# NagsTheProgrammer/WindGNN

Hardware: AMD Instinct MI355X
Metric: windows/sec (fwd+bwd) 34-node seq24 GCN-GRU (higher is better)
Workload: dtype f16x3(split-fp32); 1 GPU; S=34 stations, T=24, F=13, H=102, B=4096 windows/GPU; step = forward + MSE + backward + grad all-reduce (N>1) + Adam; fp32 I/O; global_batch=4096, parallelism=dp1, math=f16x3, collective=none (one rank)

## Files before the change

windgnn_amd/csrc/api.hip:

```cpp
#include <atomic>
#include <cmath>
#include <cstdlib>
#include <mutex>

#include "common.h"
#include "../../include/windgnn_optim.h"
#include "../../include/windgnn_sched.h"

namespace {

inline size_t rup(size_t x, size_t a) { return (x + a - 1) / a * a; }

struct Layout {
  size_t BT, I, Ip, G3, Gp, H, Hp;
  size_t Id;
  int np_g3, np_i;
  size_t ws_GI, ws_g, ws_planes_f, ws_Ylast, ws_xtail_f, ws_xtail_b, fwd_floats;
  size_t st_g, st_gates, st_yp, stash_floats;
  size_t ws_dGI, ws_dGH, ws_dg, ws_part_ih, ws_part_hh, ws_gcnpart, ws_planes_b, ws_scales, ws_dY, bwd_floats;
  size_t prep_f, prep_b, prep_floats;
  int prep_kind;
  int sk_ih, sk_hh;
  bool tn_merge;
  bool x3, gen_gcn, gen_gru, g32, g32tn;
// ... 400 lines not shown
}

int fwd_recurrence(const Fwd& f) {
  const wgnn_dims* d = f.d;
  const FwdCall& c = f.c;
  const Layout& L = f.L;
  const wgnn_params* p = c.p;
  const float y_mul = c.wind_max - c.wind_min, y_add = c.wind_min;
  const bool hn_only = c.state && !f.Y;
  float* Y = (float*)f.Y;
  const void* labels = f.sf ? c.labels : nullptr;
  float* stats = f.sf ? f.sf + L.st_stats : nullptr;
  float* hprev = (f.sf && (L.g32tn || c.sst)) ? f.sf + L.st_hprev : nullptr;
  int rc;
  if (L.x3 && !L.gen_gru) {
    if (c.last)
      return launch_grux_fwd(d->B, d->T, d->H, f.GI, (int)L.Gp, p->w_hh, p->b_hh, c.last, nullptr, nullptr, f.full, f.status,
                             nullptr, nullptr, 0, 1, y_mul, y_add, f.st);
    if (c.state) {
      const int lo = hn_only && d->io == WGNN_IO_F32;
      return launch_grux_fwd(d->B, d->T, d->H, f.GI, (int)L.Gp, p->w_hh, p->b_hh, lo ? (void*)c.hn : f.Y, nullptr, nullptr,
                             f.full, f.status, nullptr, nullptr, d->io, lo, 1.f, 0.f, f.st, c.h0, lo ? nullptr : c.hn);
    }
    rc = launch_grux_fwd(d->B, d->T, d->H, f.GI, (int)L.Gp, p->w_hh, p->b_hh, f.Y, f.gates, f.sf ? f.sf + L.st_yp : nullptr,
                         f.full, f.status, labels, stats, d->io, 0, 1.f, 0.f, f.st, c.h0, c.hn, c.sst ? L.plane_rows : 0);
  } else if (L.rec32) {
    if (c.last)
      return launch_gru_fwd(d->B, d->T, d->H, f.GI, (int)L.Gp, p->w_hh, p->b_hh, c.last, nullptr, nullptr, nullptr, nullptr, 0,
                            1, y_mul, y_add, f.st);
    if (c.state)
      return launch_gru_fwd(d->B, d->T, d->H, f.GI, (int)L.Gp, p->w_hh, p->b_hh, hn_only ? c.hn : Y, nullptr, nullptr, nullptr,
                            nullptr, 0, hn_only ? 1 : 0, 1.f, 0.f, f.st, c.h0, hn_only ? nullptr : c.hn);
    rc = launch_gru_fwd(d->B, d->T, d->H, f.GI, (int)L.Gp, p->w_hh, p->b_hh, Y, f.gates, (const float*)labels, stats, hprev,
                        L.hq, 0, 1.f, 0.f, f.st, c.h0, c.hn);
  } else if (L.small) {
    rc = launch_gru_small_fwd(d->B, d->T, d->H, f.GI, (int)L.Gp, p->w_hh, p->b_hh, Y, f.gates, hprev, L.hq,
                              (const float*)labels, stats, f.st, c.h0, c.hn);
  } else if (L.x3) {
    rc = launch_split_weight2(p->w_hh, (int)L.G3, (int)L.H, 0, p->b_hh, (int)L.H, f.ws + L.ws_hhp_f, L.np_g3, (int)L.Hp,
                              f.status, f.st);
    if (rc == WGNN_OK)
      rc = launch_gru_gen_fwd_x3(d->B, d->T, d->H, f.GI, (int)L.Gp, f.ws + L.ws_hhp_f, L.np_g3, p->b_hh, Y, f.gates,
                                 f.sf ? f.sf + L.st_yp : f.ws + L.ws_yp, f.ws + L.ws_gh, f.ws + L.ws_kp_f, f.ws + L.ws_hc,
                                 f.full, f.st, c.h0, c.sst ? L.plane_rows : 0);
  } else {
    rc = launch_gru_gen_fwd(d->B, d->T, d->H, f.GI, (int)L.Gp, p->w_hh, p->b_hh, Y, f.gates, f.ws + L.ws_gh, f.st, c.h0);
  }
  if (rc != WGNN_OK) return rc;
// ... 133 lines not shown
  if (L.gen_gru)
    return launch_gru_gen_bwd(d->B, d->T, d->H, p->w_hh, b.Y, dY, gates, b.dGI, b.dGH, (int)L.Gp, b.ws + L.ws_dhz,
                              b.ws + L.ws_dhw, b.st, sb);
  if (L.small)
    return launch_gru_small_bwd(d->B, d->T, d->H, p->w_hh, b.Y, b.fused_loss ? nullptr : dY, b.fused_loss ? labels : nullptr,
                                gates, b.dGI, b.dGH, (int)L.Gp, stats, (int64_t)L.BT * L.H, c.grad_scale, c.loss, b.status,
                                b.st, sb);
  return launch_gru_bwd(d->B, d->T, d->H, p->w_hh, b.Y, b.fused_loss ? nullptr : dY, b.fused_loss ? labels : nullptr, gates,
                        b.sf + L.st_GI, (int)L.Gp, b.dGI, (int)L.Gp, L.dghn ? b.dGH : nullptr, L.dghn ? nullptr : b.dGH, stats,
                        (int64_t)L.BT * L.H, c.grad_scale, c.loss, b.status, b.st, sb);
}

int bwd_weights(const Bwd& b, int prods, int r0, int rows) {
  const wgnn_dims* d = b.d;
  const Layout& L = b.L;
  float* part_ih = b.ws + L.ws_part_ih;
  float* part_hh = b.ws + L.ws_part_hh;
  const bool sst = b.c.sst;
  int rc = WGNN_OK;
  if (L.x3) {
    const _Float16* dGIh = (const _Float16*)b.dGI + r0;
    const _Float16* dGHh = (const _Float16*)b.dGH + r0;
    const _Float16* gh = (const _Float16*)b.gact;
    const _Float16* yph = (const _Float16*)(b.sf + L.st_yp);
    const _Float16* ypl = yph + L.plane_rows * L.Hp;
    const size_t PG = L.BT * L.Gp;
    TnProd hh = {};
    hh.lda = (int)L.Gp; hh.Bhi = yph; hh.Blo = ypl; hh.ldb = (int)L.Hp; hh.shift_T = d->T; hh.splitk = L.sk_hh;
    hh.partial = part_hh; hh.Nout = (int)L.H + 1; hh.x3 = b.full; hh.per_window = sst;
    if (L.dghn) {
      hh.Ahi = dGIh; hh.Alo = L.dgi1 ? nullptr : dGIh + PG; hh.Mout = L.m_hh;
      hh.A2hi = dGHh; hh.A2lo = L.dgi1 ? nullptr : dGHh + L.BT * (size_t)L.hn; hh.lda2 = L.hn; hh.msplit = L.msplit;
      hh.b_stream = true;
    } else {
      hh.Ahi = dGHh; hh.Alo = L.gen2p ? nullptr : dGHh + PG; hh.Mout = rows;
    }
    const bool one_pass_ih = L.dgi1 || L.gen2p;
    TnProd ih = {};
    ih.Ahi = dGIh; ih.Alo = one_pass_ih ? dGIh : dGIh + PG; ih.lda = (int)L.Gp;
    ih.Bhi = gh; ih.Blo = gh + L.BT * L.Ip; ih.ldb = (int)L.Ip; ih.splitk = L.sk_ih;
    ih.partial = part_ih; ih.Mout = rows; ih.Nout = (int)L.I + 1; ih.x3 = b.full && !one_pass_ih; ih.b_stream = true;
    auto one = [&](const TnProd& p) {
      return launch_pgemm_tn(p.Ahi, p.Alo, p.lda, p.Bhi, p.Blo, p.ldb, p.shift_T, (int)L.BT, p.splitk, p.partial, p.Mout, p.Nout,
                             p.x3, p.A2hi, p.A2lo, p.lda2, p.msplit, b.st, p.b_stream, p.per_window);
    };
    if (prods == (WGNN_ROWS_IH | WGNN_ROWS_HH) && L.tn_merge && opt(WGNN_OPT_TN_MERGED) && pgemm_tn2_covers(ih, hh)) {
      rc = launch_pgemm_tn2(ih, hh, (int)L.BT, b.st);
    } else {
      if (prods & WGNN_ROWS_HH) {
        rc = one(hh);
        if (rc != WGNN_OK) return rc;
      }
      if (prods & WGNN_ROWS_IH) rc = one(ih);
    }
  } else {
    const float* hp = b.sf + L.st_hprev;
    if (prods & WGNN_ROWS_HH) {
      if (L.g32tn && L.dghn)
        rc = launch_gemm32_tn(b.dGI, (int)L.Gp, hp, L.hq, (int)L.BT, L.sk_hh, part_hh, L.m_hh, (int)L.H + 1, b.dGH, L.hn,
                              L.msplit, b.st);
      else if (L.g32tn)
        rc = launch_gemm32_tn(b.dGH, (int)L.Gp, hp, L.hq, (int)L.BT, L.sk_hh, part_hh, rows, (int)L.H + 1, nullptr, 0, 0, b.st);
      else {
        GemmArgs a = {};
        a.A = b.dGH + r0; a.lda = (int)L.Gp; a.a_kcontig = 0;
        a.B = b.Y; a.ldb = (int)L.H; a.b_kcontig = 0; a.ones_col = 1; a.shift_T = d->T;
        if (sst) { a.B = hp; a.ldb = L.hq; a.shift_T = 0; }
        a.M = rows; a.N = (int)L.H + 1; a.K = (int)L.BT;
        a.splitk = L.sk_hh; a.partial = part_hh;
        rc = launch_gemm_f32(a, b.st);
// ... 110 lines not shown

int rows_align(const wgnn_dims* d, const Layout& L) {
  if (!L.gen_gru || d->math == WGNN_MATH_F16) return 0;
  return L.x3 ? TN_BM : 128;
}

int check_rows(const wgnn_dims* d, const Layout& L, int which, int row0, int rows) {
  if ((which & ~(WGNN_ROWS_IH | WGNN_ROWS_HH | WGNN_ROWS_STATE)) != 0 ||
      ((which & 3) != WGNN_ROWS_IH && (which & 3) != WGNN_ROWS_HH))
    return WGNN_ERR_SHAPE;
  if (which & WGNN_ROWS_STATE) return WGNN_ERR_UNSUPPORTED;
  const int al = rows_align(d, L);
  if (al == 0) return WGNN_ERR_UNSUPPORTED;
  const int64_t end = (int64_t)row0 + rows;
  if (row0 < 0 || rows < 1 || end > (int64_t)L.G3 || row0 % al != 0 || (end % al != 0 && end != (int64_t)L.G3))
    return WGNN_ERR_SHAPE;
  return WGNN_OK;
}

}

int opt_big_gemm() { return opt(WGNN_OPT_BIG_GEMM); }

int series_plan(const wgnn_dims* df, const wgnn_dims* dr, SeriesPlan* sp) {
  int rc = check_dims(df);
  if (rc == WGNN_OK) rc = check_dims(dr);
  if (rc != WGNN_OK) return rc;
  const Layout Lf = make_layout(df, false, SER_FRONT), Lr = make_layout(dr, false, SER_REC);
  if ((int64_t)Lf.BT * (int64_t)Lf.Gp >= (1ll << 31)) return WGNN_ERR_SHAPE;
  sp->ws_front = Lf.fwd_floats > Lf.bwd_floats ? Lf.fwd_floats : Lf.bwd_floats;
  sp->ws_rec = Lr.fwd_floats > Lr.bwd_floats ? Lr.fwd_floats : Lr.bwd_floats;
  sp->st_front = Lf.stash_floats;
  sp->st_rec = Lr.stash_floats;
  sp->st_g = Lf.BT * Lf.Ip; sp->st_GI = Lf.BT * Lf.Gp;
  sp->st_gates = gru_gates_floats(dr->B, dr->T, dr->H);
  sp->st_hprev = Lr.g32tn ? Lr.BT * (size_t)Lr.hq : 0;
  return WGNN_OK;
}

namespace {

int series_forward(const wgnn_dims* df, const wgnn_dims* dr, int stride, const float* A, const float* Xs, const wgnn_params* p,
                   float* Y, float* last, float wind_min, float wind_max, void* stash, void* workspace, const SeriesPlan& sp,
                   void* stream, const float* Ls, int64_t ls_rows, float* loss_buf, const int* starts) {
  const int last_start = df->T - dr->T;
  const Layout Lf = make_layout(df, false, SER_FRONT), Lr = make_layout(dr, false, SER_REC);
// ... 449 lines not shown
```

windgnn_amd/csrc/common.h:

```cpp
#pragma once
#include <hip/hip_runtime.h>
#include <stdint.h>

#include "../../include/windgnn.h"

typedef float f32x4 __attribute__((ext_vector_type(4)));
typedef float f32x16 __attribute__((ext_vector_type(16)));

#define WGNN_WAVE 64

static inline int cdiv_i(int a, int b) { return (a + b - 1) / b; }
static inline size_t align_up(size_t x, size_t a) { return (x + a - 1) / a * a; }

#define WGNN_CHECK_LAUNCH()                              \
  do {                                                   \
    if (hipGetLastError() != hipSuccess) return WGNN_ERR_HIP; \
  } while (0)

__device__ __forceinline__ f32x4 mfma16(float a, float b, f32x4 c) {
  return __builtin_amdgcn_mfma_f32_16x16x4f32(a, b, c, 0, 0, 0);
}
__device__ __forceinline__ f32x16 mfma32(float a, float b, f32x16 c) {
  return __builtin_amdgcn_mfma_f32_32x32x2f32(a, b, c, 0, 0, 0);
}
// ... 117 lines not shown
                     hipStream_t st);
int launch_gcnx2_bwd(int ntiles, int S, const float* A, const void* X, int io, const float* W1, const float* b1,
                     const float* W2, const void* g_planes, int ldg, const void* dg, int ld_dg ,
                     bool dg16 , const float* scales, int scale_in, float* partial, bool x3,
                     void* xtail_scratch, hipStream_t st);
bool gcngi_supported(int S, int H, bool x3);
int launch_gcngi_fwd(int ntiles, int S, const float* A, const void* X, int io, const float* W1, const float* b1,
                     const float* W2, const float* b2, void* g_planes, int ldg, int stash_planes, const void* Bplanes,
                     int Np, void* GI, int ldgi, int N, bool x3, unsigned* status, void* xtail_scratch, hipStream_t st);
bool gcn_any_supported(int S, int Fi, int Fo);
size_t gcn_any_bwd_partial_floats(int ntiles, int Fi, int Fo);
int launch_gcn_any_fwd(int ntiles, int S, int Fi, int Fo, const float* A, const float* X, const float* W, const float* b, float* out,
                       hipStream_t st);
int launch_gcn_any_bwd(int ntiles, int S, int Fi, int Fo, const float* A, const float* X, const float* W, const float* out,
                       const float* dout, float* dW, float* db, float* dX, float* partial, hipStream_t st);
int launch_pack_g(const float* gin, size_t rows, int I, float* g, int ld, hipStream_t st);
int launch_unpack_dg(const float* dg, size_t rows, int I, int ld, float* out, hipStream_t st);
bool pgemm_nt256_wanted(int M, int N, int Kp);
int launch_pgemm_nt256(const void* Aimg_hi, const void* Aimg_lo, int M, int k0, int klen, const void* Bplanes, int Np,
                       size_t bplane, float* C, int ldc, int N, bool accumulate, hipStream_t st);
size_t pgemm_nt256_aimg_bytes(int M, int N, int Kp, int planes);
int launch_pgemm_repack_a(const void* Ahi, const void* Alo, int lda, int M, int Kp, void* img, hipStream_t st);
int opt_big_gemm();
__host__ __device__ __forceinline__ size_t bimg_off(int n, int k, int Np) {
  return ((size_t)(k >> 5) * (size_t)(Np >> 4) + (size_t)(n >> 4)) * 512 + (size_t)(((k >> 3) & 3) * 128 + (n & 15) * 8 + (k & 7));
}
int launch_split_weight2(const float* W, int R, int C, int transpose, const float* bias, int bias_col, void* planes,
                         int Rp, int Cp, unsigned* status, hipStream_t st);
int pgemm_nt_np(int N);
int pgemm_tn_tiles(int Mout, int Nout);
size_t pgemm_tn_partial_floats(int Mout, int Nout, int splitk);
size_t pgemm_nt_kpart_floats(int M, int ldc, int Kp);
int launch_pgemm_nt(const void* Ahi, const void* Alo, int lda, int M, int Kp, const void* Bplanes, int Np, float* C,
                    int ldc, int N, const float* s_out, bool x3, float* kpart, hipStream_t st, bool out16 = false,
                    void* aimg = nullptr );
int launch_pgemm_tn(const void* Ahi, const void* Alo, int lda, const void* Bhi, const void* Blo, int ldb, int shift_T,
                    int K, int splitk, float* partial, int Mout, int Nout, bool x3, const void* A2hi, const void* A2lo,
                    int lda2, int msplit, hipStream_t st, bool b_stream = false ,
                    bool per_window = false );
struct TnProd {
  const void *Ahi, *Alo; int lda;
  const void *Bhi, *Blo; int ldb;
  int shift_T, splitk;
  float* partial;
  int Mout, Nout;
  bool x3;
  const void *A2hi, *A2lo; int lda2, msplit;
  bool b_stream, per_window;
};
bool pgemm_tn2_covers(const TnProd& ih, const TnProd& hh);
int launch_pgemm_tn2(const TnProd& ih, const TnProd& hh, int K, hipStream_t st);
size_t gcn_csr_bwd_partial_floats();
int launch_gcn2_csr_fwd(int ntiles, int S, int nnz, const void* csr, const float* X, const float* W1, const float* b1,
                        const float* W2, const float* b2, float* h1, float* g, void* g_planes, size_t ldg, bool x3,
                        unsigned* status, hipStream_t st);
int launch_gcn2_csr_bwd(int ntiles, int S, int nnz, const void* csr, const float* X, const float* W2, const float* h1,
                        const float* g, const void* g_hi, size_t ldg, const float* dg, size_t ld_dg,
                        const float* scales, float* du, float* partial, float* dW1, float* db1, float* dW2, float* db2,
                        hipStream_t st);
int launch_gru_gen_fwd_x3(int B, int T, int H, const float* GI, int ldgi, const void* whh_planes, int np_g3,
                          const float* bhh, float* Y, float* gates, void* y_planes, float* gh, float* kpart, void* hc,
                          bool x3, hipStream_t st, const float* h0 = nullptr,
                          size_t plane_rows = 0 );
int launch_h0_planes(int B, int H, int Hp, const float* h0, void* hi, void* lo, hipStream_t st);
int launch_gru_gen_bwd_x3(int B, int T, int H, const void* whhT_planes, int np_h, const float* Y, const float* dY,
                          const float* gates, const float* scales, void* dgi_planes, void* dgh_planes, int ldd,
                          float* dhz, float* dhw, float* kpart, void* dc, bool x3, hipStream_t st,
                          const BwdState* state = nullptr);
int launch_gru_gen_fwd(int B, int T, int H, const float* GI, int ldgi, const float* Whh, const float* bhh, float* Y,
                       float* gates, float* gh, hipStream_t st, const float* h0 = nullptr);
int launch_gru_gen_bwd(int B, int T, int H, const float* Whh, const float* Y, const float* dY, const float* gates,
                       float* dGI, float* dGH, int ldd, float* dhz, float* dhw, hipStream_t st,
                       const BwdState* state = nullptr);
// ... 137 lines not shown
```

windgnn_amd/csrc/pgemm.hip:

```cpp
#include <string>

#include "common.h"

typedef _Float16 h8 __attribute__((ext_vector_type(8)));
typedef _Float16 h4 __attribute__((ext_vector_type(4)));
typedef __fp16 fh4 __attribute__((__vector_size__(4 * sizeof(__fp16))));
typedef unsigned int u32x4 __attribute__((ext_vector_type(4)));

namespace {

constexpr int NT_BM = 192, NT_WAVES = 12;

__device__ __forceinline__ int swz16(int row) { return (4 - (row >> 2)) & 3; }
__device__ __forceinline__ int sw16_off(int row, int c) { return row * 64 + ((c ^ swz16(row)) << 4); }

__device__ __forceinline__ f32x4 mfma_q(h8 a, h8 b, f32x4 c) {
  return __builtin_amdgcn_mfma_f32_16x16x32_f16(a, b, c, 0, 0, 0);
}

constexpr int nt_a_slot(bool x3, bool alo) { return ((x3 && alo) ? 2 : 1) * NT_BM * 64; }
constexpr int nt_b_slot(int T, bool x3) { return (x3 ? 2 : 1) * 32 * T * 64; }
constexpr int nt_a_depth(int T, bool x3, bool alo) {
  return (!x3 && 3 * nt_a_slot(x3, alo) + 2 * nt_b_slot(T, x3) <= 156 * 1024) ? 3 : 2;
}
constexpr size_t nt_smem(int T, bool x3, bool alo) {
  return (size_t)nt_a_depth(T, x3, alo) * nt_a_slot(x3, alo) + 2 * (size_t)nt_b_slot(T, x3);
}

template <int T, bool X3, bool ALO, bool OUT16>
__global__ void __launch_bounds__(64 * NT_WAVES) pgemm_nt_kernel(const _Float16* __restrict__ Ahi,
                                                                const _Float16* __restrict__ Alo, int lda, int M,
                                                                int Kp, const _Float16* __restrict__ Bpl, int Np,
                                                                float* __restrict__ C, int ldc, int N,
                                                                const float* __restrict__ s_out_p, int nm, int nsl,
                                                                size_t bplane, int kc_len, int kc_first,
                                                                size_t cstride, int accumulate) {
  {
    const int k0 = (kc_first + (int)blockIdx.y) * kc_len;
    Ahi += k0;
    Alo += k0;
// ... 217 lines not shown
  for (int j = 0; j < T; ++j) {
    const int col = n0 + BNW * wn + 16 * j + r16;
    if (col >= N) continue;
#pragma unroll
    for (int i = 0; i < 2; ++i)
#pragma unroll
      for (int r = 0; r < 4; ++r) {
        const int row = m0 + 32 * wm + 16 * i + 4 * c4 + r;
        if (row < M) {
          float* dst = C + (size_t)row * ldc + col;
          const float v = acc[i][j][r] * s_out;
          *dst = accumulate ? *dst + v : v;
        }
      }
  }
}


__device__ __forceinline__ int tn_g(int stride32, int r) {
  const int u = stride32 & 7;
  return u == 0 ? (r & 7) : (u == 4 ? ((r >> 1) & 3) : ((r >> 2) & 1));
}

template <int T, bool X3, bool A2, bool ALO, bool PW = false>
__device__ __forceinline__ void pgemm_tn_tile(const _Float16* __restrict__ Ahi, const _Float16* __restrict__ Alo, int lda,
                                              const _Float16* __restrict__ Bhi, const _Float16* __restrict__ Blo, int ldb,
                                              int shift_T, int K, int kchunk, float* __restrict__ partial, int Mout,
                                              int Nout, int nNb, const _Float16* __restrict__ A2hi,
                                              const _Float16* __restrict__ A2lo, int lda2, int msplit, int b_stream,
                                              const int z, const int tile, const int ntile) {
  constexpr int BM = TN_BM, BN = 32 * T;
  constexpr int ARB = BM * 2, BRB = BN * 2;
  constexpr int A_PL = 32 * ARB, B_PL = 32 * BRB, STAGE = 2 * A_PL + 2 * B_PL;
  constexpr int PL = X3 ? 2 : 1;
  constexpr int PLA = (X3 && ALO) ? 2 : 1;
  constexpr int AP = A_PL / 1024, BP = B_PL / 1024;
  constexpr int NPIECE = PLA * AP + PL * BP, NIT = (NPIECE + TN_WAVES - 1) / TN_WAVES;
  constexpr int ACH = ARB / 16, BCH = BRB / 16;
  extern __shared__ __attribute__((aligned(16))) char smem[];
  const int tid = threadIdx.x, lane = tid & 63;
  const int wave = __builtin_amdgcn_readfirstlane(tid >> 6);
  const int wm = wave & 3, wn = wave >> 2;
  const int mb = tile / nNb, nb = tile % nNb;
  const int m0 = mb * BM, n0 = nb * BN;
  const int kbeg = z * kchunk, kend = min(K, kbeg + kchunk);
  const int nk = kend > kbeg ? (kend - kbeg + 31) / 32 : 0;

  f32x4 acc[5][T];
#pragma unroll
  for (int i = 0; i < 5; ++i)
#pragma unroll
    for (int j = 0; j < T; ++j) acc[i][j] = f32x4{0.f, 0.f, 0.f, 0.f};

  const _Float16* base[NIT];
  int ld[NIT], dst[NIT], prow[NIT], pcol[NIT];
  bool on[NIT], isb[NIT];
#pragma unroll
  for (int it = 0; it < NIT; ++it) {
    const int p = wave + TN_WAVES * it;
    on[it] = p < NPIECE;
    const int pp = on[it] ? p : 0;
    isb[it] = pp >= PLA * AP;
    if (!isb[it]) {
      const int plane = pp / AP, q = 64 * (pp % AP) + lane;
      const int row = q / ACH, pos = q % ACH;
      const int col = m0 + 8 * (pos ^ (2 * tn_g(ARB / 32, row)));
      base[it] = plane ? Alo : Ahi;
      ld[it] = lda;
      prow[it] = row;
      pcol[it] = col < lda ? col : 0;
      if (A2 && col >= msplit) {
        base[it] = plane ? A2lo : A2hi;
        ld[it] = lda2;
        pcol[it] = col - msplit < lda2 ? col - msplit : 0;
      }
      dst[it] = plane * A_PL + (pp % AP) * 1024;
    } else {
      const int q2 = pp - PLA * AP;
      const int plane = q2 / BP, q = 64 * (q2 % BP) + lane;
      const int row = q / BCH, pos = q % BCH;
      const int col = n0 + 8 * (pos ^ (2 * tn_g(BRB / 32, row)));
      base[it] = plane ? Blo : Bhi;
      ld[it] = ldb;
      prow[it] = row;
      pcol[it] = col < ldb ? col : 0;
      dst[it] = 2 * A_PL + plane * B_PL + (q2 % BP) * 1024;
    }
  }
  typedef __attribute__((address_space(3))) void lds_void;
  typedef __attribute__((address_space(1))) const void glb_void;
  auto dma_stage = [&](char* st, int k0) {
#pragma unroll
    for (int it = 0; it < NIT; ++it)
      if (on[it]) {
        int k = min(k0 + prow[it], kend - 1);
        if (isb[it] && shift_T > 0) k = (k % shift_T) != 0 ? k - 1 : (PW ? K + k / shift_T : K);
        if (isb[it] && b_stream)
          __builtin_amdgcn_global_load_lds((glb_void*)(base[it] + (size_t)k * ld[it] + pcol[it]),
                                           (lds_void*)(st + dst[it]), 16, 0, 2);
        else
          __builtin_amdgcn_global_load_lds((glb_void*)(base[it] + (size_t)k * ld[it] + pcol[it]),
                                           (lds_void*)(st + dst[it]), 16, 0, 0);
      }
  };

  const int x = lane >> 4, q4 = (lane & 15) >> 2, p4 = lane & 3;
  const int r1 = 4 * x + q4;
  const int gA = 2 * tn_g(ARB / 32, r1), gB = 2 * tn_g(BRB / 32, r1);
  int a_off[5], b_off[T];
#pragma unroll
  for (int i = 0; i < 5; ++i) a_off[i] = r1 * ARB + 16 * ((2 * (5 * wm + i) + (p4 >> 1)) ^ gA) + 8 * (p4 & 1);
#pragma unroll
  for (int j = 0; j < T; ++j)
    b_off[j] = 2 * A_PL + r1 * BRB + 16 * ((2 * (T * wn + j) + (p4 >> 1)) ^ gB) + 8 * (p4 & 1);
  typedef __attribute__((address_space(3))) fh4 lds_fh4;
  auto trread = [&](const char* p0, int rb) -> h8 {
    const fh4 v0 = __builtin_amdgcn_ds_read_tr16_b64_v4f16((lds_fh4*)p0);
    const fh4 v1 = __builtin_amdgcn_ds_read_tr16_b64_v4f16((lds_fh4*)(p0 + 16 * rb));
    const h4 w0 = __builtin_bit_cast(h4, v0), w1 = __builtin_bit_cast(h4, v1);
    h8 r;
    r[0] = w0[0]; r[1] = w0[1]; r[2] = w0[2]; r[3] = w0[3];
    r[4] = w1[0]; r[5] = w1[1]; r[6] = w1[2]; r[7] = w1[3];
    return r;
  };
  auto compute = [&](const char* cur) {
    h8 ah[5], al[5];
#pragma unroll
    for (int i = 0; i < 5; ++i) {
      ah[i] = trread(cur + a_off[i], ARB);
      al[i] = ah[i];
      if (X3 && ALO) al[i] = trread(cur + A_PL + a_off[i], ARB);
    }
#pragma unroll
    for (int j = 0; j < T; ++j) {
      const h8 bh = trread(cur + b_off[j], BRB);
      if (X3) {
        const h8 bl = trread(cur + B_PL + b_off[j], BRB);
#pragma unroll
        for (int i = 0; i < 5; ++i) {
          if (ALO) acc[i][j] = mfma_q(al[i], bh, acc[i][j]);
          acc[i][j] = mfma_q(ah[i], bl, acc[i][j]);
        }
      }
#pragma unroll
      for (int i = 0; i < 5; ++i) acc[i][j] = mfma_q(ah[i], bh, acc[i][j]);
    }
  };

  if (nk > 0) dma_stage(smem, kbeg);
  for (int kt = 0; kt < nk; ++kt) {
    char* cur = smem + (kt & 1) * STAGE;
    asm volatile("s_waitcnt vmcnt(0)" ::: "memory");
    __builtin_amdgcn_s_barrier();
    if (kt + 1 < nk) dma_stage(smem + ((kt + 1) & 1) * STAGE, kbeg + 32 * (kt + 1));
    const int rows = kend - (kbeg + 32 * kt);
    if (rows < 32) {
      const u32x4 zero = {0u, 0u, 0u, 0u};
      for (int c = tid; c < (32 - rows) * ACH; c += 64 * TN_WAVES) {
        *(u32x4*)(cur + rows * ARB + 16 * c) = zero;
        if (X3 && ALO) *(u32x4*)(cur + A_PL + rows * ARB + 16 * c) = zero;
      }
      __syncthreads();
    }
    compute(cur);
  }

  float* P = partial + (((size_t)z * ntile + tile) * TN_WAVES + wave) * (5 * T * 256) + lane * 4;
#pragma unroll
  for (int i = 0; i < 5; ++i)
#pragma unroll
    for (int j = 0; j < T; ++j) {
      *(f32x4*)(P + (i * T + j) * 256) = acc[i][j];
    }
}

template <int T, bool X3, bool A2, bool ALO, bool PW = false>
__global__ void __launch_bounds__(64 * TN_WAVES) pgemm_tn_kernel(const _Float16* __restrict__ Ahi,
                                                                const _Float16* __restrict__ Alo, int lda,
                                                                const _Float16* __restrict__ Bhi,
                                                                const _Float16* __restrict__ Blo, int ldb,
                                                                int shift_T, int K, int kchunk,
                                                                float* __restrict__ partial, int Mout, int Nout,
                                                                int nNb, const _Float16* __restrict__ A2hi,
                                                                const _Float16* __restrict__ A2lo, int lda2,
                                                                int msplit, int b_stream) {
  pgemm_tn_tile<T, X3, A2, ALO, PW>(Ahi, Alo, lda, Bhi, Blo, ldb, shift_T, K, kchunk, partial, Mout, Nout, nNb, A2hi, A2lo,
                                    lda2, msplit, b_stream, (int)blockIdx.x, (int)blockIdx.y, (int)gridDim.y);
}

struct TnRole {
  const _Float16 *Ahi, *Alo, *Bhi, *Blo, *A2hi, *A2lo;
  float* partial;
  int lda, ldb, lda2, shift_T, K, kchunk, Mout, Nout, nNb, msplit, b_stream, splitk, ntile;
};
template <int TI, int TH, int MODE, bool PW>
__global__ void __launch_bounds__(64 * TN_WAVES) pgemm_tn2_kernel(const TnRole ih, const TnRole hh) {
  const int item = (int)blockIdx.x;
  if (item < ih.splitk * ih.ntile)
    pgemm_tn_tile<TI, MODE == 0, false, true, false>(ih.Ahi, ih.Alo, ih.lda, ih.Bhi, ih.Blo, ih.ldb, ih.shift_T, ih.K, ih.kchunk,
                                                     ih.partial, ih.Mout, ih.Nout, ih.nNb, ih.A2hi, ih.A2lo, ih.lda2, ih.msplit,
                                                     ih.b_stream, item % ih.splitk, item / ih.splitk, ih.ntile);
  __syncthreads();
  if (item < hh.splitk * hh.ntile)
    pgemm_tn_tile<TH, MODE != 2, true, MODE != 1, PW>(hh.Ahi, hh.Alo, hh.lda, hh.Bhi, hh.Blo, hh.ldb, hh.shift_T, hh.K, hh.kchunk,
                                                      hh.partial, hh.Mout, hh.Nout, hh.nNb, hh.A2hi, hh.A2lo, hh.lda2, hh.msplit,
                                                      hh.b_stream, item % hh.splitk, item / hh.splitk, hh.ntile);
}

__global__ void split_weight2_kernel(const float* __restrict__ W, int R, int C, int transpose,
                                     const float* __restrict__ bias, int bias_col, _Float16* hi, _Float16* lo,
                                     int Rp, int Cp, unsigned* status) {
  typedef _Float16 h8v __attribute__((ext_vector_type(8)));
  const size_t pi = (size_t)blockIdx.x * blockDim.x + threadIdx.x;
  if (pi >= (size_t)Rp * Cp / 8) return;
  const int tile = (int)(pi >> 6), within = (int)(pi & 63);
  const int kt = tile / (Rp >> 4), nt = tile % (Rp >> 4);
  const int r = 16 * nt + (within & 15), c0 = 32 * kt + 8 * (within >> 4);
  float v[8];
  if (transpose) {
#pragma unroll
    for (int k = 0; k < 8; ++k) v[k] = (c0 + k < R && r < C) ? W[(size_t)(c0 + k) * C + r] : 0.f;
  } else if (r < R && c0 + 7 < C && (((size_t)r * C + c0) & 3) == 0) {
    const f32x4 a = *(const f32x4*)(W + (size_t)r * C + c0), b = *(const f32x4*)(W + (size_t)r * C + c0 + 4);
#pragma unroll
    for (int k = 0; k < 4; ++k) { v[k] = a[k]; v[4 + k] = b[k]; }
  } else {
#pragma unroll
    for (int k = 0; k < 8; ++k) {
      const int c = c0 + k;
// ... 238 lines not shown
  case t: return launch_tn_t<t>(Ahi, Alo, lda, Bhi, Blo, ldb, shift_T, K, splitk, partial, Mout, Nout, x3, nNb, A2hi, A2lo, \
                                lda2, msplit, st, b_stream, per_window);
    TN_CASE(1) TN_CASE(2) TN_CASE(3) TN_CASE(4) TN_CASE(5) TN_CASE(6) TN_CASE(7)
#undef TN_CASE
  }
  return WGNN_ERR_SHAPE;
}

namespace {
int tn2_mode(const TnProd& ih, const TnProd& hh) {
  const bool ih3 = ih.x3 && ih.Alo, hh3 = hh.x3 && hh.Alo, hh2 = hh.x3 && !hh.Alo;
  if (ih3 && hh3) return 0;
  if (!ih.x3 && hh2) return 1;
  if (!ih.x3 && !hh.x3) return 2;
  return -1;
}

template <int TI, int TH>
int launch_tn2_t(const TnProd& pi, const TnProd& ph, int K, int mode, int nNi, int nNh, hipStream_t st) {
  auto role = [K](const TnProd& p, int nNb) {
    TnRole r;
    const bool alo = p.Alo != nullptr;
    r.Ahi = (const _Float16*)p.Ahi; r.Alo = (const _Float16*)(alo ? p.Alo : p.Ahi);
    r.Bhi = (const _Float16*)p.Bhi; r.Blo = (const _Float16*)p.Blo;
    r.A2hi = (const _Float16*)p.A2hi; r.A2lo = (const _Float16*)(alo ? p.A2lo : p.A2hi);
    r.partial = p.partial;
    r.lda = p.lda; r.ldb = p.ldb; r.lda2 = p.lda2; r.shift_T = p.shift_T; r.K = K;
    r.kchunk = cdiv_i(cdiv_i(K, p.splitk), 32) * 32;
    r.Mout = p.Mout; r.Nout = p.Nout; r.nNb = nNb; r.msplit = p.msplit; r.b_stream = p.b_stream ? 1 : 0;
    r.splitk = p.splitk; r.ntile = cdiv_i(p.Mout, TN_BM) * nNb;
    return r;
  };
  const TnRole ri = role(pi, nNi), rh = role(ph, nNh);
  constexpr int TMAX = TI > TH ? TI : TH;
  const size_t smem = 2 * (size_t)(2 * 32 * 2 * (TN_BM + 32 * TMAX));
  auto bytes = [K](const TnProd& p) {
    return ((p.x3 && p.Alo) ? 4.0 : 2.0) * (double)K * p.Mout + (p.x3 ? 4.0 : 2.0) * (double)K * p.Nout +
           4.0 * (double)p.splitk * p.Mout * p.Nout;
  };
  const double fl = 2.0 * K * ((double)pi.Mout * pi.Nout + (double)ph.Mout * ph.Nout), by = bytes(pi) + bytes(ph);
  static const std::string base = "pgemm_tn_kernel<" + std::to_string(TI) + "+" + std::to_string(TH);
  static const std::string names[3] = {base + ">", base + ",x2>", base + ",f16>"};
  const int ni = ri.splitk * ri.ntile, nh = rh.splitk * rh.ntile;
  const dim3 grid(ni > nh ? ni : nh), block(64 * TN_WAVES);
#define TN2_GO(MODE, PWV)                                                                                        \
  do {                                                                                                           \
    static std::atomic<unsigned long long> done_{0};                                                             \
    if (ensure_dyn_smem((const void*)pgemm_tn2_kernel<TI, TH, MODE, PWV>, smem, done_) != WGNN_OK) return WGNN_ERR_HIP; \
    PROF_LAUNCH(names[MODE].c_str(), fl, by, st,                                                                 \
                hipLaunchKernelGGL((pgemm_tn2_kernel<TI, TH, MODE, PWV>), grid, block, smem, st, ri, rh));       \
  } while (0)
  switch (2 * mode + (ph.per_window ? 1 : 0)) {
    case 0: TN2_GO(0, false); break;
    case 1: TN2_GO(0, true); break;
    case 2: TN2_GO(1, false); break;
    case 3: TN2_GO(1, true); break;
    case 4: TN2_GO(2, false); break;
    case 5: TN2_GO(2, true); break;
    default: return WGNN_ERR_UNSUPPORTED;
  }
#undef TN2_GO
  WGNN_CHECK_LAUNCH();
  return WGNN_OK;
}
}

bool pgemm_tn2_covers(const TnProd& ih, const TnProd& hh) {
  int nNb, T;
  tn_shape(hh.Nout, nNb, T);
  return tn2_mode(ih, hh) >= 0 && !ih.A2hi && ih.shift_T == 0 && !ih.per_window && hh.A2hi && T <= 4 && ih.splitk >= 1 &&
         hh.splitk >= 1;
}

int launch_pgemm_tn2(const TnProd& ih, const TnProd& hh, int K, hipStream_t st) {
  if (!pgemm_tn2_covers(ih, hh)) return WGNN_ERR_UNSUPPORTED;
  if (ih.lda % 8 != 0 || ih.ldb % 8 != 0 || hh.lda % 8 != 0 || hh.ldb % 8 != 0 || K < 1) return WGNN_ERR_SHAPE;
  if (hh.per_window && hh.shift_T < 1) return WGNN_ERR_SHAPE;
  if (hh.lda2 % 8 != 0 || hh.msplit % 8 != 0 || hh.msplit > hh.lda) return WGNN_ERR_SHAPE;
  int nNi, TI, nNh, TH;
  tn_shape(ih.Nout, nNi, TI);
  tn_shape(hh.Nout, nNh, TH);
  const int mode = tn2_mode(ih, hh);
  switch (4 * (TI - 1) + (TH - 1)) {
#define TN2_CASE(ti, th) \
  case 4 * (ti - 1) + (th - 1): return launch_tn2_t<ti, th>(ih, hh, K, mode, nNi, nNh, st);
#define TN2_ROW(ti) TN2_CASE(ti, 1) TN2_CASE(ti, 2) TN2_CASE(ti, 3) TN2_CASE(ti, 4)
    TN2_ROW(1) TN2_ROW(2) TN2_ROW(3) TN2_ROW(4) TN2_ROW(5) TN2_ROW(6) TN2_ROW(7)
#undef TN2_ROW
#undef TN2_CASE
  }
  return WGNN_ERR_SHAPE;
}
```

windgnn_amd/functional.py:

```python
from __future__ import annotations

import ctypes as C
from typing import Sequence

import torch

from . import _lib

PARAM_ORDER = ("conv1.weight", "conv1.bias", "conv2.weight", "conv2.bias",
               "gru.weight_ih_l0", "gru.weight_hh_l0", "gru.bias_ih_l0", "gru.bias_hh_l0")


_IO_OF = {torch.float32: _lib.IO_F32, torch.float16: _lib.IO_F16, torch.bfloat16: _lib.IO_BF16}


def _require_gpu(*tensors: torch.Tensor, io_ok: bool = False) -> None:
    for t in tensors:
        if not t.is_cuda:
            raise RuntimeError(
                "windgnn_amd runs on an MI355X (HIP) only: got a %s tensor. There is no CPU fallback; "
                "use the oracle under oracle/ for CPU checks." % t.device)
        if t.dtype != torch.float32 and not (io_ok and t.dtype in _IO_OF):
            raise RuntimeError("windgnn_amd: expected float32 tensors, got %s" % t.dtype)

# ... 142 lines not shown
    _require_gpu(*params)
    _require_contiguous(X=X, labels=labels, params=params)
    if X.dim() != 4:
        raise RuntimeError("windgnn_amd: X must be [B, T, S, 13], got %s" % (tuple(X.shape),))
    BX, T, S, F = X.shape
    B = BX if B is None else B
    A, fmt, nnz = _adj(A, S)
    H = params[5].shape[1]
    for name, t in (("h0", h0), ("h_n", h_n)):
        if t is None:
            continue
        _require_gpu(t)
        _require_contiguous(**{name: t})
        if tuple(t.shape) != (B, H) or t.device != X.device:
            raise RuntimeError("windgnn_amd: %s must be [B, H] = [%d, %d] float32 on %s, got %s on %s"
                               % (name, B, H, X.device, tuple(t.shape), t.device))
    d = _lib.Dims(B, T, S, F, H, math, fmt, nnz, _IO_OF[X.dtype])
    ws, ws_bytes = _workspace(d, X.device, refused="wgnn_workspace_bytes(B=%d,T=%d,S=%d,F=%d,H=%d,math=%d,io=%s)"
                              % (B, T, S, F, H, math, X.dtype))
    return A, d, ws, ws_bytes


def gcn_gru_forward_raw(A, X, params: Sequence[torch.Tensor], math=_lib.MATH_F32, want_stash=True, labels=None,
                        prepared=None):
    lib = _lib.load()
    A, d, ws, ws_bytes = _forward_setup(A, X, params, math, labels=labels)
    B, T, H = d.B, d.T, d.H
    stash = torch.empty(lib.wgnn_stash_bytes(C.byref(d)), dtype=torch.uint8, device=X.device) if want_stash else None
    Y = torch.empty(B, T, H, dtype=X.dtype, device=X.device)
    ps = _params_struct(_lib.Params, params, prepared)
    if labels is not None:
        _require_gpu(labels, io_ok=True)
        if labels.dtype != X.dtype:
            raise RuntimeError("windgnn_amd: labels are %s but X is %s (one I/O type per call)" % (labels.dtype, X.dtype))
        if labels.numel() != Y.numel() or not want_stash:
            raise RuntimeError("windgnn_amd: wgnn_fwd_loss needs a stash and labels of Y's size, got %s vs %s"
                               % (tuple(labels.shape), tuple(Y.shape)))
        rc = lib.wgnn_fwd_loss(C.byref(d), _ptr(A), _ptr(X), C.byref(ps), _ptr(labels), _ptr(Y),
                               _stash_ptr(stash), _ptr(ws), ws_bytes, _stream())
        _lib.check(rc, "wgnn_fwd_loss")
        return Y, stash, d
    rc = lib.wgnn_fwd(C.byref(d), _ptr(A), _ptr(X), C.byref(ps), _ptr(Y), _stash_ptr(stash), _ptr(ws), ws_bytes, _stream())
    _lib.check(rc, "wgnn_fwd")
    return Y, stash, d


def gcn_gru_state(A, X, params: Sequence[torch.Tensor], math=_lib.MATH_F32, h0=None, want_y=True, h_n=None):
    lib = _lib.load()
    A, d, ws, ws_bytes = _forward_setup(A, X, params, math, h0=h0, h_n=h_n)
    B, T, H = d.B, d.T, d.H
    Y = torch.empty(B, T, H, dtype=X.dtype, device=X.device) if want_y else None
# ... 404 lines not shown
```

Before: 5.666 million windows/s.

## Feed hh weight-gradient GEMM directly from fp32 Y, skipping split-plane stash

In the x3 (split-fp16) path the forward GRU no longer writes hi/lo fp16 planes of the previous hidden state into the stash when an env-controlled condition holds. The merged TN weight-gradient kernel instead DMAs fp32 Y rows into LDS, applies a per-row time-shift mask, and splits them into hi/lo fp16 in registers before the MFMAs. This removes a stash write and read of two fp16 planes, at the cost of extra in-kernel conversion work and more complex load addressing. The Python API also gains an optional preallocated stash argument.

```diff
diff --git a/windgnn_amd/csrc/api.hip b/windgnn_amd/csrc/api.hip
--- a/windgnn_amd/csrc/api.hip
+++ b/windgnn_amd/csrc/api.hip
@@ -446,8 +446,9 @@
       return launch_grux_fwd(d->B, d->T, d->H, f.GI, (int)L.Gp, p->w_hh, p->b_hh, lo ? (void*)c.hn : f.Y, nullptr, nullptr,
                              f.full, f.status, nullptr, nullptr, d->io, lo, 1.f, 0.f, f.st, c.h0, lo ? nullptr : c.hn);
     }
-    rc = launch_grux_fwd(d->B, d->T, d->H, f.GI, (int)L.Gp, p->w_hh, p->b_hh, f.Y, f.gates, f.sf ? f.sf + L.st_yp : nullptr,
-                         f.full, f.status, labels, stats, d->io, 0, 1.f, 0.f, f.st, c.h0, c.hn, c.sst ? L.plane_rows : 0);
+    rc = launch_grux_fwd(d->B, d->T, d->H, f.GI, (int)L.Gp, p->w_hh, p->b_hh, f.Y, f.gates,
+                         f.sf && !hh_from_y(d, L.tn_merge, c.sst) ? f.sf + L.st_yp : nullptr, f.full, f.status, labels, stats,
+                         d->io, 0, 1.f, 0.f, f.st, c.h0, c.hn, c.sst ? L.plane_rows : 0);
   } else if (L.rec32) {
     if (c.last)
       return launch_gru_fwd(d->B, d->T, d->H, f.GI, (int)L.Gp, p->w_hh, p->b_hh, c.last, nullptr, nullptr, nullptr, nullptr, 0,
@@ -627,8 +628,7 @@
     const _Float16* dGIh = (const _Float16*)b.dGI + r0;
     const _Float16* dGHh = (const _Float16*)b.dGH + r0;
     const _Float16* gh = (const _Float16*)b.gact;
-    const _Float16* yph = (const _Float16*)(b.sf + L.st_yp);
-    const _Float16* ypl = yph + L.plane_rows * L.Hp;
+    const _Float16 *yph = (const _Float16*)(b.sf + L.st_yp), *ypl = yph + L.plane_rows * L.Hp;
     const size_t PG = L.BT * L.Gp;
     TnProd hh = {};
     hh.lda = (int)L.Gp; hh.Bhi = yph; hh.Blo = ypl; hh.ldb = (int)L.Hp; hh.shift_T = d->T; hh.splitk = L.sk_hh;
@@ -650,7 +650,7 @@
                              p.x3, p.A2hi, p.A2lo, p.lda2, p.msplit, b.st, p.b_stream, p.per_window);
     };
     if (prods == (WGNN_ROWS_IH | WGNN_ROWS_HH) && L.tn_merge && opt(WGNN_OPT_TN_MERGED) && pgemm_tn2_covers(ih, hh)) {
-      rc = launch_pgemm_tn2(ih, hh, (int)L.BT, b.st);
+      rc = launch_pgemm_tn2(ih, tn_b_from_y(hh, hh_from_y(d, L.tn_merge, sst) ? b.Y : nullptr, (int)L.H), (int)L.BT, b.st);
     } else {
       if (prods & WGNN_ROWS_HH) {
         rc = one(hh);
@@ -807,6 +807,11 @@
 
 int opt_big_gemm() { return opt(WGNN_OPT_BIG_GEMM); }
 
+bool hh_from_y(const wgnn_dims* d, bool tn_merge, bool sst) {
+  static const int from_env = env_int("WGNN_TN_YFP32", 1, 0, 1);
+  return tn_merge && three_pass(d) && d->io == WGNN_IO_F32 && !sst && from_env && opt(WGNN_OPT_TN_MERGED);
+}
+
 int series_plan(const wgnn_dims* df, const wgnn_dims* dr, SeriesPlan* sp) {
   int rc = check_dims(df);
   if (rc == WGNN_OK) rc = check_dims(dr);
diff --git a/windgnn_amd/csrc/common.h b/windgnn_amd/csrc/common.h
--- a/windgnn_amd/csrc/common.h
+++ b/windgnn_amd/csrc/common.h
@@ -163,6 +163,7 @@
 size_t pgemm_nt256_aimg_bytes(int M, int N, int Kp, int planes);
 int launch_pgemm_repack_a(const void* Ahi, const void* Alo, int lda, int M, int Kp, void* img, hipStream_t st);
 int opt_big_gemm();
+bool hh_from_y(const wgnn_dims* d, bool tn_merge, bool sst);
 __host__ __device__ __forceinline__ size_t bimg_off(int n, int k, int Np) {
   return ((size_t)(k >> 5) * (size_t)(Np >> 4) + (size_t)(n >> 4)) * 512 + (size_t)(((k >> 3) & 3) * 128 + (n & 15) * 8 + (k & 7));
 }
@@ -188,8 +189,10 @@
   bool x3;
   const void *A2hi, *A2lo; int lda2, msplit;
   bool b_stream, per_window;
+  const float* By;
 };
 bool pgemm_tn2_covers(const TnProd& ih, const TnProd& hh);
+TnProd tn_b_from_y(TnProd hh, const float* Y, int H);
 int launch_pgemm_tn2(const TnProd& ih, const TnProd& hh, int K, hipStream_t st);
 size_t gcn_csr_bwd_partial_floats();
 int launch_gcn2_csr_fwd(int ntiles, int S, int nnz, const void* csr, const float* X, const float* W1, const float* b1,
diff --git a/windgnn_amd/csrc/pgemm.hip b/windgnn_amd/csrc/pgemm.hip
--- a/windgnn_amd/csrc/pgemm.hip
+++ b/windgnn_amd/csrc/pgemm.hip
@@ -16,6 +16,22 @@
 
 __device__ __forceinline__ f32x4 mfma_q(h8 a, h8 b, f32x4 c) {
   return __builtin_amdgcn_mfma_f32_16x16x32_f16(a, b, c, 0, 0, 0);
+}
+
+__device__ __forceinline__ unsigned cvt2(float x0, float x1) {
+  typedef float f2v __attribute__((ext_vector_type(2)));
+  typedef _Float16 h2v __attribute__((ext_vector_type(2)));
+  const f2v xv = {x0, x1};
+  return __builtin_bit_cast(unsigned, __builtin_convertvector(xv, h2v));
+}
+__device__ __forceinline__ void split2(float x0, float x1, unsigned& hi, unsigned& lo) {
+  float t0, t1;
+  hi = cvt2(x0, x1);
+  asm("v_fma_mix_f32 %0, %2, -1.0, %3 op_sel:[0,0,0] op_sel_hi:[1,0,0]\n\t"
+      "v_fma_mix_f32 %1, %2, -1.0, %4 op_sel:[1,0,0] op_sel_hi:[1,0,0]"
+      : "=&v"(t0), "=&v"(t1)
+      : "v"(hi), "v"(x0), "v"(x1));
+  lo = cvt2(t0, t1);
 }
 
 constexpr int nt_a_slot(bool x3, bool alo) { return ((x3 && alo) ? 2 : 1) * NT_BM * 64; }
@@ -279,20 +295,22 @@
   return u == 0 ? (r & 7) : (u == 4 ? ((r >> 1) & 3) : ((r >> 2) & 1));
 }
 
-template <int T, bool X3, bool A2, bool ALO, bool PW = false>
+template <int T, bool X3, bool A2, bool ALO, bool PW = false, bool YB = false>
 __device__ __forceinline__ void pgemm_tn_tile(const _Float16* __restrict__ Ahi, const _Float16* __restrict__ Alo, int lda,
                                               const _Float16* __restrict__ Bhi, const _Float16* __restrict__ Blo, int ldb,
                                               int shift_T, int K, int kchunk, float* __restrict__ partial, int Mout,
                                               int Nout, int nNb, const _Float16* __restrict__ A2hi,
                                               const _Float16* __restrict__ A2lo, int lda2, int msplit, int b_stream,
-                                              const int z, const int tile, const int ntile) {
+                                              const int z, const int tile, const int ntile,
+                                              const float* __restrict__ By = nullptr) {
+  static_assert(!YB || (X3 && !PW), "the fp32 B source: split modes, the stateless step");
   constexpr int BM = TN_BM, BN = 32 * T;
   constexpr int ARB = BM * 2, BRB = BN * 2;
   constexpr int A_PL = 32 * ARB, B_PL = 32 * BRB, STAGE = 2 * A_PL + 2 * B_PL;
   constexpr int PL = X3 ? 2 : 1;
   constexpr int PLA = (X3 && ALO) ? 2 : 1;
   constexpr int AP = A_PL / 1024, BP = B_PL / 1024;
-  constexpr int NPIECE = PLA * AP + PL * BP, NIT = (NPIECE + TN_WAVES - 1) / TN_WAVES;
+  constexpr int NPIECE = PLA * AP + (YB ? 2 : PL) * BP, NIT = (NPIECE + TN_WAVES - 1) / TN_WAVES;
   constexpr int ACH = ARB / 16, BCH = BRB / 16;
   extern __shared__ __attribute__((aligned(16))) char smem[];
   const int tid = threadIdx.x, lane = tid & 63;
@@ -309,6 +327,11 @@
 #pragma unroll
     for (int j = 0; j < T; ++j) acc[i][j] = f32x4{0.f, 0.f, 0.f, 0.f};
 
+  const uintptr_t y_s0 = YB ? (uintptr_t)By + ((ptrdiff_t)kbeg - 1) * ldb * 4 : 0;
+  const int y_d4 = (int)(y_s0 & 15);
+  const uintptr_t y_stage = y_s0 - y_d4;
+  const uintptr_t y_lo = (uintptr_t)By & ~(uintptr_t)15, y_hi = ((uintptr_t)By + (size_t)K * ldb * 4 - 4) & ~(uintptr_t)15;
+  const int y_bytes = y_d4 + 128 * ldb;
   const _Float16* base[NIT];
   int ld[NIT], dst[NIT], prow[NIT], pcol[NIT];
   bool on[NIT], isb[NIT];
@@ -332,6 +355,14 @@
         pcol[it] = col - msplit < lda2 ? col - msplit : 0;
       }
       dst[it] = plane * A_PL + (pp % AP) * 1024;
+    } else if (YB) {
+      const int q2 = pp - PLA * AP;
+      on[it] = on[it] && q2 * 1024 < y_bytes;
+      base[it] = Bhi;
+      ld[it] = 0;
+      prow[it] = 0;
+      pcol[it] = q2 * 1024 + lane * 16;
+      dst[it] = 2 * A_PL + q2 * 1024;
     } else {
       const int q2 = pp - PLA * AP;
       const int plane = q2 / BP, q = 64 * (q2 % BP) + lane;
@@ -350,6 +381,13 @@
 #pragma unroll
     for (int it = 0; it < NIT; ++it)
       if (on[it]) {
+        if (YB && isb[it]) {
+          uintptr_t a = y_stage + (size_t)(k0 - kbeg) * ldb * 4 + pcol[it];
+          a = a < y_lo ? y_lo : (a > y_hi ? y_hi : a);
+          if (b_stream) __builtin_amdgcn_global_load_lds((glb_void*)a, (lds_void*)(st + dst[it]), 16, 0, 2);
+          else __builtin_amdgcn_global_load_lds((glb_void*)a, (lds_void*)(st + dst[it]), 16, 0, 0);
+          continue;
+        }
         int k = min(k0 + prow[it], kend - 1);
         if (isb[it] && shift_T > 0) k = (k % shift_T) != 0 ? k - 1 : (PW ? K + k / shift_T : K);
         if (isb[it] && b_stream)
@@ -380,7 +418,39 @@
     r[4] = w1[0]; r[5] = w1[1]; r[6] = w1[2]; r[7] = w1[3];
     return r;
   };
-  auto compute = [&](const char* cur) {
+  int y_off[8];
+  bool y_col[T], y_edge[T];
+  float y_pad[T];
+#pragma unroll
+  for (int e = 0; e < 8; ++e)
+    y_off[e] = 2 * A_PL + y_d4 + 4 * ((4 * x + (e & 3) + 16 * (e >> 2)) * ldb + 16 * T * wn + (lane & 15));
+#pragma unroll
+  for (int j = 0; j < T; ++j) {
+    const int c = 16 * (T * wn + j) + (lane & 15);
+    y_col[j] = c < ldb;
+    y_pad[j] = c == ldb ? 1.f : 0.f;
+    y_edge[j] = 16 * (T * wn + j) + 16 > ldb;
+  }
+  auto yfrag = [&](const char* cur, int j, const unsigned (&m)[8], h8& bh, h8& bl) {
+    float v[8];
+#pragma unroll
+    for (int e = 0; e < 8; ++e) v[e] = __builtin_bit_cast(float, *(const unsigned*)(cur + y_off[e] + 64 * j) & m[e]);
+    if (y_edge[j]) {
+#pragma unroll
+      for (int e = 0; e < 8; ++e) v[e] = y_col[j] ? v[e] : y_pad[j];
+    }
+    u32x4 hi, lo;
+#pragma unroll
+    for (int e = 0; e < 4; ++e) {
+      unsigned h, l;
+      split2(v[2 * e], v[2 * e + 1], h, l);
+      hi[e] = h;
+      lo[e] = l;
+    }
+    bh = __builtin_bit_cast(h8, hi);
+    bl = __builtin_bit_cast(h8, lo);
+  };
+  auto compute = [&](const char* cur, unsigned keep) {
     h8 ah[5], al[5];
 #pragma unroll
     for (int i = 0; i < 5; ++i) {
@@ -388,11 +458,19 @@
       al[i] = ah[i];
       if (X3 && ALO) al[i] = trread(cur + A_PL + a_off[i], ARB);
     }
+    unsigned ym[8];
+    if (YB) {
+      const unsigned sh = keep >> (4 * x);
+#pragma unroll
+      for (int e = 0; e < 8; ++e) ym[e] = 0u - ((sh >> ((e & 3) + 16 * (e >> 2))) & 1u);
+    }
 #pragma unroll
     for (int j = 0; j < T; ++j) {
-      const h8 bh = trread(cur + b_off[j], BRB);
+      h8 bh, ybl;
+      if (YB) yfrag(cur, j, ym, bh, ybl);
+      else bh = trread(cur + b_off[j], BRB);
       if (X3) {
-        const h8 bl = trread(cur + B_PL + b_off[j], BRB);
+        const h8 bl = YB ? ybl : trread(cur + B_PL + b_off[j], BRB);
 #pragma unroll
         for (int i = 0; i < 5; ++i) {
           if (ALO) acc[i][j] = mfma_q(al[i], bh, acc[i][j]);
@@ -404,6 +482,8 @@
     }
   };
 
+  int y_rem = YB ? kbeg % shift_T : 0;
+  const int y_step = YB ? 32 % shift_T : 0;
   if (nk > 0) dma_stage(smem, kbeg);
   for (int kt = 0; kt < nk; ++kt) {
     char* cur = smem + (kt & 1) * STAGE;
@@ -419,7 +499,15 @@
       }
       __syncthreads();
     }
-    compute(cur);
+    unsigned keep = 0u;
+    if (YB) {
+      unsigned t0 = 0u;
+      for (int r = y_rem ? shift_T - y_rem : 0; r < 32; r += shift_T) t0 |= 1u << r;
+      keep = ~t0 & (rows >= 32 ? ~0u : (1u << rows) - 1u);
+      y_rem += y_step;
+      if (y_rem >= shift_T) y_rem -= shift_T;
+    }
+    compute(cur, keep);
   }
 
   float* P = partial + (((size_t)z * ntile + tile) * TN_WAVES + wave) * (5 * T * 256) + lane * 4;
@@ -447,10 +535,11 @@
 
 struct TnRole {
   const _Float16 *Ahi, *Alo, *Bhi, *Blo, *A2hi, *A2lo;
+  const float* By;
   float* partial;
   int lda, ldb, lda2, shift_T, K, kchunk, Mout, Nout, nNb, msplit, b_stream, splitk, ntile;
 };
-template <int TI, int TH, int MODE, bool PW>
+template <int TI, int TH, int MODE, bool PW, bool YB = false>
 __global__ void __launch_bounds__(64 * TN_WAVES) pgemm_tn2_kernel(const TnRole ih, const TnRole hh) {
   const int item = (int)blockIdx.x;
   if (item < ih.splitk * ih.ntile)
@@ -459,9 +548,10 @@
                                                      ih.b_stream, item % ih.splitk, item / ih.splitk, ih.ntile);
   __syncthreads();
   if (item < hh.splitk * hh.ntile)
-    pgemm_tn_tile<TH, MODE != 2, true, MODE != 1, PW>(hh.Ahi, hh.Alo, hh.lda, hh.Bhi, hh.Blo, hh.ldb, hh.shift_T, hh.K, hh.kchunk,
-                                                      hh.partial, hh.Mout, hh.Nout, hh.nNb, hh.A2hi, hh.A2lo, hh.lda2, hh.msplit,
-                                                      hh.b_stream, item % hh.splitk, item / hh.splitk, hh.ntile);
+    pgemm_tn_tile<TH, MODE != 2, true, MODE != 1, PW, YB>(hh.Ahi, hh.Alo, hh.lda, hh.Bhi, hh.Blo, hh.ldb, hh.shift_T, hh.K,
+                                                          hh.kchunk, hh.partial, hh.Mout, hh.Nout, hh.nNb, hh.A2hi, hh.A2lo,
+                                                          hh.lda2, hh.msplit, hh.b_stream, item % hh.splitk, item / hh.splitk,
+                                                          hh.ntile, hh.By);
 }
 
 __global__ void split_weight2_kernel(const float* __restrict__ W, int R, int C, int transpose,
@@ -746,7 +836,7 @@
     TnRole r;
     const bool alo = p.Alo != nullptr;
     r.Ahi = (const _Float16*)p.Ahi; r.Alo = (const _Float16*)(alo ? p.Alo : p.Ahi);
-    r.Bhi = (const _Float16*)p.Bhi; r.Blo = (const _Float16*)p.Blo;
+    r.Bhi = (const _Float16*)p.Bhi; r.Blo = (const _Float16*)p.Blo; r.By = p.By;
     r.A2hi = (const _Float16*)p.A2hi; r.A2lo = (const _Float16*)(alo ? p.A2lo : p.A2hi);
     r.partial = p.partial;
     r.lda = p.lda; r.ldb = p.ldb; r.lda2 = p.lda2; r.shift_T = p.shift_T; r.K = K;
@@ -759,28 +849,30 @@
   constexpr int TMAX = TI > TH ? TI : TH;
   const size_t smem = 2 * (size_t)(2 * 32 * 2 * (TN_BM + 32 * TMAX));
   auto bytes = [K](const TnProd& p) {
-    return ((p.x3 && p.Alo) ? 4.0 : 2.0) * (double)K * p.Mout + (p.x3 ? 4.0 : 2.0) * (double)K * p.Nout +
-           4.0 * (double)p.splitk * p.Mout * p.Nout;
+    return ((p.x3 && p.Alo) ? 4.0 : 2.0) * (double)K * p.Mout +
+           (p.By ? 4.0 * (double)K * p.ldb : (p.x3 ? 4.0 : 2.0) * (double)K * p.Nout) + 4.0 * (double)p.splitk * p.Mout * p.Nout;
   };
   const double fl = 2.0 * K * ((double)pi.Mout * pi.Nout + (double)ph.Mout * ph.Nout), by = bytes(pi) + bytes(ph);
   static const std::string base = "pgemm_tn_kernel<" + std::to_string(TI) + "+" + std::to_string(TH);
   static const std::string names[3] = {base + ">", base + ",x2>", base + ",f16>"};
   const int ni = ri.splitk * ri.ntile, nh = rh.splitk * rh.ntile;
   const dim3 grid(ni > nh ? ni : nh), block(64 * TN_WAVES);
-#define TN2_GO(MODE, PWV)                                                                                        \
+#define TN2_GO(MODE, PWV, YBV)                                                                                   \
   do {                                                                                                           \
     static std::atomic<unsigned long long> done_{0};                                                             \
-    if (ensure_dyn_smem((const void*)pgemm_tn2_kernel<TI, TH, MODE, PWV>, smem, done_) != WGNN_OK) return WGNN_ERR_HIP; \
+    if (ensure_dyn_smem((const void*)pgemm_tn2_kernel<TI, TH, MODE, PWV, YBV>, smem, done_) != WGNN_OK) return WGNN_ERR_HIP; \
     PROF_LAUNCH(names[MODE].c_str(), fl, by, st,                                                                 \
-                hipLaunchKernelGGL((pgemm_tn2_kernel<TI, TH, MODE, PWV>), grid, block, smem, st, ri, rh));       \
+                hipLaunchKernelGGL((pgemm_tn2_kernel<TI, TH, MODE, PWV, YBV>), grid, block, smem, st, ri, rh));  \
   } while (0)
-  switch (2 * mode + (ph.per_window ? 1 : 0)) {
-    case 0: TN2_GO(0, false); break;
-    case 1: TN2_GO(0, true); break;
-    case 2: TN2_GO(1, false); break;
-    case 3: TN2_GO(1, true); break;
-    case 4: TN2_GO(2, false); break;
-    case 5: TN2_GO(2, true); break;
+  switch (2 * mode + (ph.per_window ? 1 : 0) + (ph.By ? 6 : 0)) {
+    case 0: TN2_GO(0, false, false); break;
+    case 1: TN2_GO(0, true, false); break;
+    case 2: TN2_GO(1, false, false); break;
+    case 3: TN2_GO(1, true, false); break;
+    case 4: TN2_GO(2, false, false); break;
+    case 5: TN2_GO(2, true, false); break;
+    case 6: TN2_GO(0, false, true); break;
+    case 8: TN2_GO(1, false, true); break;
     default: return WGNN_ERR_UNSUPPORTED;
   }
 #undef TN2_GO
@@ -792,13 +884,20 @@
 bool pgemm_tn2_covers(const TnProd& ih, const TnProd& hh) {
   int nNb, T;
   tn_shape(hh.Nout, nNb, T);
-  return tn2_mode(ih, hh) >= 0 && !ih.A2hi && ih.shift_T == 0 && !ih.per_window && hh.A2hi && T <= 4 && ih.splitk >= 1 &&
-         hh.splitk >= 1;
+  if (hh.By && (tn2_mode(ih, hh) > 1 || hh.per_window || hh.shift_T < 1 || nNb != 1 || hh.ldb + 1 != hh.Nout)) return false;
+  return tn2_mode(ih, hh) >= 0 && !ih.By && !ih.A2hi && ih.shift_T == 0 && !ih.per_window && hh.A2hi && T <= 4 &&
+         ih.splitk >= 1 && hh.splitk >= 1;
+}
+
+TnProd tn_b_from_y(TnProd hh, const float* Y, int H) {
+  if (Y) { hh.By = Y; hh.ldb = H; hh.Bhi = hh.Blo = nullptr; }
+  return hh;
 }
 
 int launch_pgemm_tn2(const TnProd& ih, const TnProd& hh, int K, hipStream_t st) {
   if (!pgemm_tn2_covers(ih, hh)) return WGNN_ERR_UNSUPPORTED;
-  if (ih.lda % 8 != 0 || ih.ldb % 8 != 0 || hh.lda % 8 != 0 || hh.ldb % 8 != 0 || K < 1) return WGNN_ERR_SHAPE;
+  if (ih.lda % 8 != 0 || ih.ldb % 8 != 0 || hh.lda % 8 != 0 || (!hh.By && hh.ldb % 8 != 0) || K < 1) return WGNN_ERR_SHAPE;
+  if (hh.By && ((uintptr_t)hh.By & 3)) return WGNN_ERR_SHAPE;
   if (hh.per_window && hh.shift_T < 1) return WGNN_ERR_SHAPE;
   if (hh.lda2 % 8 != 0 || hh.msplit % 8 != 0 || hh.msplit > hh.lda) return WGNN_ERR_SHAPE;
   int nNi, TI, nNh, TH;
diff --git a/windgnn_amd/functional.py b/windgnn_amd/functional.py
--- a/windgnn_amd/functional.py
+++ b/windgnn_amd/functional.py
@@ -188,11 +188,16 @@
 
 
 def gcn_gru_forward_raw(A, X, params: Sequence[torch.Tensor], math=_lib.MATH_F32, want_stash=True, labels=None,
-                        prepared=None):
+                        prepared=None, stash=None):
     lib = _lib.load()
     A, d, ws, ws_bytes = _forward_setup(A, X, params, math, labels=labels)
     B, T, H = d.B, d.T, d.H
-    stash = torch.empty(lib.wgnn_stash_bytes(C.byref(d)), dtype=torch.uint8, device=X.device) if want_stash else None
+    if stash is not None:
+        if not want_stash or stash.dtype != torch.uint8 or stash.device != X.device or stash.numel() < lib.wgnn_stash_bytes(C.byref(d)):
+            raise RuntimeError("windgnn_amd: stash must be a uint8 buffer of wgnn_stash_bytes = %d bytes on %s"
+                               % (lib.wgnn_stash_bytes(C.byref(d)), X.device))
+    elif want_stash:
+        stash = torch.empty(lib.wgnn_stash_bytes(C.byref(d)), dtype=torch.uint8, device=X.device)
     Y = torch.empty(B, T, H, dtype=X.dtype, device=X.device)
     ps = _params_struct(_lib.Params, params, prepared)
     if labels is not None:
```

Result: faster. 5.756 million windows/s, median of 6 (+1.6%).
